# halajun/diasss

Hardware: AMD Instinct MI355X
Metric: sonar frames/sec end-to-end (extract+match+LM solve) (higher is better)
Workload: dtype u8/int32 (extract, match) + f64 (geo gate, LM); 1 GPU; 200 synthetic 2000x1024 frames, dense all-pairs; frames=200, pings=2000, bins=1024, pairs=19900

## Files before the change

diasss_amd/csrc/dsss_ctx.hip:

```cpp
#include "dsss_internal.h"
#include "dsss_pg_sym.h"
#include <algorithm>
#include <chrono>
#include <thread>
#include <atomic>
#include <cstdlib>

void dsss_prof_flush(dsss_ctx* c)
{
    if (!c || c->prof.pending.empty()) return;
    hipStreamSynchronize(c->stream);
    for (const dsss_prof::rec& r : c->prof.pending) {
        float ms = 0;
        if (hipEventElapsedTime(&ms, r.e0, r.e1) == hipSuccess) { c->prof.ms[r.k] += ms; c->prof.launches[r.k] += r.nl; }
        c->prof.pool.push_back(r.e0); c->prof.pool.push_back(r.e1);
    }
    c->prof.pending.clear();
}

dsss_switches dsss_switches_read()
{
    dsss_switches sw;
    if (const char* v = getenv("DSSS_EX_SCRATCH_MB")) sw.ex_scratch_mb = (size_t)std::max(1, atoi(v));
    if (const char* v = getenv("DSSS_EX_UPLOAD_BATCH")) sw.ex_upload_batch = std::max(1, atoi(v));
    sw.ex_verbose = getenv("DSSS_EX_VERBOSE") != nullptr;
    if (const char* v = getenv("DSSS_FS_THREADS")) sw.fs_threads = atoi(v);
    if (const char* v = getenv("DSSS_MT_GRID")) sw.mt_grid = atoi(v) != 0;
    sw.sift_hist_dump = getenv("DSSS_SIFT_HIST_DUMP");
    if (const char* v = getenv("DSSS_REG_PEAKS")) sw.reg_peaks_host = strcmp(v, "host") == 0;
    return sw;
}

extern "C" {

void dsss_mask_params_default(dsss_mask_params* p) { p->factor = 2.5; p->width = 10; p->r = 6; p->side = 150; }
void dsss_orb_params_default(dsss_orb_params* p) { p->nfeatures = 2000; p->scale = 1.2f; p->nlevels = 6; p->ini_th = 12; p->min_th = 7; p->descriptor = DSSS_DESC_ORB; }
void dsss_match_params_default(dsss_match_params* p)
{
    p->use_l2 = 0; p->radius = 8; p->bound_same = 88; p->bound_diff = 80; p->l2_bound = 350; p->ratio = 0.35;
    p->scc_iters = 1000; p->pix_err = 2.5; p->merge_thr = 2.5;
}
void dsss_pg_params_default(dsss_pg_params* p)
{
    p->max_iters = 100; p->rel_tol = 1e-5; p->abs_tol = 1e-5; p->lambda0 = 1e-5; p->lambda_factor = 10;
    p->lambda_max = 1e5; p->min_fidelity = 1e-3; p->add_noise = 1;
}

const char* dsss_strerror(int code)
{
    switch (code) {
    case DSSS_OK: return "ok";
    case DSSS_E_NODEVICE: return "no HIP device (libdsss has no CPU fallback)";
    case DSSS_E_ARG: return "bad argument";
    case DSSS_E_HIP: return "HIP runtime error";
    case DSSS_E_STATE: return "call order violated";
    case DSSS_E_CAPACITY: return "buffer too small";
    case DSSS_E_NUMERIC: return "numerical failure";
    case DSSS_E_COMM: return "communicator / RCCL failure";
    default: return "unknown error";
    }
}
const char* dsss_last_error(const dsss_ctx* c) { return c ? c->err.c_str() : "null context"; }

static int kcap_for(const dsss_orb_params& op) { return ((op.nfeatures + 3 * op.nlevels + 63) / 64 + 1) * 64; }

int dsss_create(int device, int max_frames, dsss_ctx** out)
{
    if (!out || max_frames <= 0) return DSSS_E_ARG;
    int ndev = 0;
    if (hipGetDeviceCount(&ndev) != hipSuccess || ndev <= 0 || device < 0 || device >= ndev) return DSSS_E_NODEVICE;
    if (hipSetDevice(device) != hipSuccess) return DSSS_E_NODEVICE;
    dsss_ctx* c = new dsss_ctx();
    c->device = device;
    dsss_mask_params_default(&c->mp); dsss_orb_params_default(&c->op);
    dsss_match_params_default(&c->mt); dsss_pg_params_default(&c->pg);
    c->max_frames = max_frames;
    c->frames.resize(max_frames);
    c->kcap = kcap_for(c->op);
    if (hipStreamCreateWithFlags(&c->stream, hipStreamNonBlocking) != hipSuccess) { delete c; return DSSS_E_HIP; }
    hipEventCreate(&c->prof.e0); hipEventCreate(&c->prof.e1);
    int prio_lo = 0, prio_hi = 0;
    (void)hipDeviceGetStreamPriorityRange(&prio_lo, &prio_hi);
    for (int i = 0; i < 4; ++i) {
        if (i == 1 && prio_hi != prio_lo) { if (hipStreamCreateWithPriority(&c->xs[i], hipStreamNonBlocking, prio_hi) != hipSuccess) { (void)hipGetLastError(); c->xs[i] = nullptr; } }
        if (!c->xs[i]) hipStreamCreateWithFlags(&c->xs[i], hipStreamNonBlocking);
        hipEventCreateWithFlags(&c->xev[i], hipEventDisableTiming);
    }
    for (int i = 0; i < DSSS_MAX_LEVELS; ++i) { hipEventCreateWithFlags(&c->ex_lev_ev[i], hipEventDisableTiming); hipEventCreateWithFlags(&c->ex_cmp_ev[i], hipEventDisableTiming); }
    for (int i = 0; i < 3; ++i) hipEventCreateWithFlags(&c->ex_side_ev[i], hipEventDisableTiming);
    hipEventCreateWithFlags(&c->xev_main, hipEventDisableTiming);
    *out = c;
    return DSSS_OK;
}

static std::array<dsss_fam_slot, 2> pack_family(dsss_frame& f, size_t pack = 0) { return {{ dsss_slot(f.d_pack, pack * sizeof(double)), dsss_slot(f.h_pack, pack * sizeof(double), DSSS_PINNED) }}; }
static std::array<dsss_fam_slot, 2> gbatch_family(dsss_geo_batch& G, size_t total = 0) { return {{ dsss_slot(G.d, total * sizeof(double)), dsss_slot(G.h, total * sizeof(double), DSSS_PINNED) }}; }
static std::array<dsss_fam_slot, 7> store_family(dsss_ctx* c)
{
    const size_t F = (size_t)c->max_frames, K = (size_t)c->kcap;
    return {{ dsss_slot(c->kps, F * K * sizeof(dsss_kp)), dsss_slot(c->desc, F * K * 32), dsss_slot(c->geo, F * K * 2 * sizeof(double)), dsss_slot(c->nkp_dev, F * sizeof(int)),
              dsss_slot(c->rows_dev, F * sizeof(int)), dsss_slot(c->cols_dev, F * sizeof(int)), dsss_slot(c->bbox_dev, F * 4 * sizeof(double)) }};
}

static void free_frame(dsss_frame& f)
{
    dsss_family_release(f.pack_cap, pack_family(f));
    hipFree(f.mask);
    if (f.pack_ev) hipEventDestroy(f.pack_ev);
    for (int l = 0; l < DSSS_MAX_LEVELS; ++l) hipFree(f.lvl[l]);
    const unsigned long long epoch = f.epoch;
    f = dsss_frame();
    f.epoch = epoch;
// ... 720 lines not shown
```

diasss_amd/csrc/dsss_internal.h:

```cpp
#pragma once
#include <hip/hip_runtime.h>
#include <cstdint>
#include <cstdio>
#include <cstring>
#include <cmath>
#include <cassert>
#include <array>
#include <string>
#include <utility>
#include <vector>
#include "../../include/dsss.h"

#define DSSS_MAX_LEVELS 8
#define DSSS_PI_REF 3.14159265359

struct dsss_ctx;
int dsss_hip_fail(dsss_ctx* c, hipError_t e, const char* file, int line, const char* call);
int dsss_alloc_fail(dsss_ctx* c, hipError_t e, const char* name, const char* step, size_t bytes);

inline hipError_t dsss_mem_alloc(void** p, size_t bytes, bool pinned) { return pinned ? hipHostMalloc(p, bytes, hipHostMallocDefault) : hipMalloc(p, bytes); }
inline void dsss_mem_free(void* p, bool pinned) { if (p) { if (pinned) (void)hipHostFree(p); else (void)hipFree(p); } }

struct dsss_buf {
    void* p = nullptr; size_t cap = 0; const char* const name; const bool pinned;
// ... 140 lines not shown
    dsss_prof prof;
};

#define DSSS_FAIL(ctx, code, ...) do { char _b[512]; snprintf(_b, sizeof _b, __VA_ARGS__); (ctx)->err = _b; return (code); } while (0)
#define HIPCHK(ctx, call) do { hipError_t _e = (call); if (_e != hipSuccess) return dsss_hip_fail((ctx), _e, __FILE__, __LINE__, #call); } while (0)
inline int dsss_hip_fail(dsss_ctx* c, hipError_t e, const char* file, int line, const char* call)
{
    char b[512]; snprintf(b, sizeof b, "%s:%d %s -> %s", file, line, call, hipGetErrorString(e));
    c->err = b; return DSSS_E_HIP;
}

inline int dsss_alloc_fail(dsss_ctx* c, hipError_t e, const char* name, const char* step, size_t bytes)
{
    char b[512]; snprintf(b, sizeof b, "%s: %s (%zu bytes) -> %s", name, step, bytes, hipGetErrorString(e));
    c->err = b; return DSSS_E_HIP;
}

inline int dsss_buf::reserve(dsss_ctx* c, size_t need_bytes, size_t alloc_bytes)
{
    if (cap >= need_bytes) return DSSS_OK;
    hipError_t e = p ? hipStreamSynchronize(c->stream) : hipSuccess;
    if (e != hipSuccess) { release(); return dsss_alloc_fail(c, e, name, "hipStreamSynchronize before the old block goes", alloc_bytes); }
    release();
    void* q = nullptr;
    if ((e = dsss_mem_alloc(&q, alloc_bytes, pinned)) != hipSuccess) return dsss_alloc_fail(c, e, name, pinned ? "hipHostMalloc" : "hipMalloc", alloc_bytes);
    p = q; cap = alloc_bytes;
    return DSSS_OK;
}
inline int dsss_buf::reserve_keep(dsss_ctx* c, size_t need_bytes, size_t alloc_bytes, size_t keep_bytes)
{
    if (cap >= need_bytes) return DSSS_OK;
    hipError_t e = p ? hipStreamSynchronize(c->stream) : hipSuccess;
    if (e != hipSuccess) return dsss_alloc_fail(c, e, name, "hipStreamSynchronize before the old block goes", alloc_bytes);
    dsss_buf nw(name, pinned);
    if ((e = dsss_mem_alloc(&nw.p, alloc_bytes, pinned)) != hipSuccess) { nw.p = nullptr; return dsss_alloc_fail(c, e, name, pinned ? "hipHostMalloc" : "hipMalloc", alloc_bytes); }
    nw.cap = alloc_bytes;
    if (keep_bytes > 0 && p && (e = hipMemcpy(nw.p, p, keep_bytes, hipMemcpyDeviceToDevice)) != hipSuccess) return dsss_alloc_fail(c, e, name, "copy of the kept prefix", keep_bytes);
    *this = std::move(nw);
    return DSSS_OK;
}
template <class Fam> int dsss_family_alloc(dsss_ctx* c, const char* name, size_t& cap, size_t new_cap, const Fam& fam)
{
    bool any = false;
    for (const dsss_fam_slot& s : fam) any = any || *s.pp != nullptr;
    hipError_t e = any ? hipStreamSynchronize(c->stream) : hipSuccess;
    dsss_family_release(cap, fam);
    if (e != hipSuccess) return dsss_alloc_fail(c, e, name, "hipStreamSynchronize before the old blocks go", 0);
    for (const dsss_fam_slot& s : fam) {
        void* q = nullptr;
        if ((e = dsss_mem_alloc(&q, s.bytes, s.pinned)) != hipSuccess) { dsss_family_release(cap, fam); return dsss_alloc_fail(c, e, name, s.pinned ? "hipHostMalloc" : "hipMalloc", s.bytes); }
        *s.pp = q;
    }
    cap = new_cap;
    return DSSS_OK;
}

struct dsss_scope {
    dsss_ctx* c; int k; int nl; hipEvent_t e0 = nullptr, e1 = nullptr;
    static hipEvent_t take(dsss_ctx* c) {
        hipEvent_t e = nullptr;
        if (!c->prof.pool.empty()) { e = c->prof.pool.back(); c->prof.pool.pop_back(); } else hipEventCreate(&e);
        return e;
    }
    dsss_scope(dsss_ctx* c_, int k_, double work = 0, int launches = 1) : c(c_), k(k_), nl(launches) {
        if (c->prof.on) { c->prof.work[k] += work; e0 = take(c); e1 = take(c); hipEventRecord(e0, c->stream); }
    }
    ~dsss_scope() {
        if (e0) {
            hipEventRecord(e1, c->stream);
            c->prof.pending.push_back({ k, nl, e0, e1 });
            if (c->prof.pending.size() >= 16384) dsss_prof_flush(c);
        }
    }
};

struct dsss_switches {
    size_t ex_scratch_mb = 24576;
    int ex_upload_batch = 8;
    bool ex_verbose = false;
    int fs_threads = 0;
    bool mt_grid = true;
    const char* sift_hist_dump = nullptr;
    bool reg_peaks_host = false;
};
dsss_switches dsss_switches_read();

void dsss_extract_eager(dsss_ctx* c, const int* ids, int n, const dsss_switches& sw);
int dsss_ensure_store(dsss_ctx* c);
int dsss_ensure_sift_store(dsss_ctx* c);
struct ex_frame;
void dsss_launch_sift_desc(dsss_ctx* c, hipStream_t st, const ex_frame* d_exf, int kcap, int nb, const char* hist_dump);
int dsss_frame_geo_bbox(dsss_ctx* c, int id);
int dsss_bboxes_enqueue(dsss_ctx* c);
int dsss_sync_bboxes(dsss_ctx* c);
int dsss_frame_kp_geo(dsss_ctx* c, int id, int n);
int dsss_mt_reserve_pair_index(dsss_ctx* c, size_t npairs);
int dsss_mt_reserve_pair_match(dsss_ctx* c, size_t npairs);
int dsss_mt_reserve_rows(dsss_ctx* c, size_t n);
int dsss_mt_upload_ptr_tables(dsss_ctx* c);
void dsss_mt_clear_results(dsss_ctx* c);
void dsss_mt_free(dsss_ctx* c);
void dsss_pg_free(dsss_ctx* c);
void dsss_comm_free(dsss_ctx* c);
void dsss_canvas_free_all(dsss_ctx* c);
int dsss_comm_rank(const dsss_ctx* c);
int dsss_comm_world(const dsss_ctx* c);
int dsss_comm_allreduce(dsss_ctx* c, double* dev, size_t n, hipStream_t st);
int dsss_comm_allgather(dsss_ctx* c, void* recv_dev, size_t bytes_per_rank, hipStream_t st);

__host__ __device__ inline void dsss_sincos(double x, double* s, double* c)
{
    const double invpio2 = 6.36619772367581382433e-01;
    const double pio2_1 = 1.57079632673412561417e+00;
    const double pio2_1t = 6.07710050650619224932e-11;
    double k = rint(x * invpio2);
    double r = (x - k * pio2_1) - k * pio2_1t;
    double z = r * r;
    double ps = 1.58969099521155010221e-10;
    ps = ps * z + -2.50507602534068634195e-08;
    ps = ps * z + 2.75573137070700676789e-06;
    ps = ps * z + -1.98412698298579493134e-04;
    ps = ps * z + 8.33333333332248946124e-03;
    ps = ps * z + -1.66666666666666324348e-01;
    double sr = r + (r * z) * ps;
    double pc = -1.13596475577881948265e-11;
    pc = pc * z + 2.08757232129817482790e-09;
    pc = pc * z + -2.75573143513906633035e-07;
    pc = pc * z + 2.48015872894767294178e-05;
    pc = pc * z + -1.38888888888741095749e-03;
    pc = pc * z + 4.16666666666666019037e-02;
    double cr = (1.0 - 0.5 * z) + (z * z) * pc;
    long long q = ((long long)k) & 3;
    if (q == 0) { *s = sr; *c = cr; }
    else if (q == 1) { *s = cr; *c = -sr; }
    else if (q == 2) { *s = -sr; *c = -cr; }
    else { *s = -cr; *c = sr; }
}

__host__ __device__ inline void dsss_geo_side(const double* P, bool starboard, double* s, double* c)
{
    dsss_sincos(starboard ? P[2] + DSSS_PI_REF / 2 : P[2] - DSSS_PI_REF / 2, s, c);
}
__host__ __device__ inline int dsss_geo_index(int M, int col)
{
    int half = M / 2, idx;
    if (col >= half) idx = col - half;
    else { idx = half - col; if (idx > half - 1) idx = half - 1; }
    return idx;
}
__host__ __device__ inline void dsss_geo_bin(const double* P, const double* gr, int M, int col, double s, double c, double* x, double* y)
{
    const int idx = dsss_geo_index(M, col);
    *x = (P[3] - 0.0) + gr[idx] * c;
    *y = (P[4] - 0.0) + gr[idx] * s;
}
__host__ __device__ inline void dsss_geo_at(const double* pose6, const double* gr, int M, int row, int col,
                                            double* x, double* y)
{
    const double* P = pose6 + (size_t)row * 6;
    double s, c;
    dsss_geo_side(P, col >= M / 2, &s, &c);
    dsss_geo_bin(P, gr, M, col, s, c, x, y);
}
__host__ __device__ inline void dsss_rotate_row(const double* row, double cx, double cy, double theta, double s, double c, double* out)
{
    out[0] = row[0]; out[1] = row[1]; out[5] = row[5];
// ... 8 lines not shown
```

diasss_amd/csrc/dsss_lc.hip:

```cpp
#include "dsss_internal.h"
#include "dsss_pose.h"
#include "dsss_lm.h"
#include <algorithm>

#define MR 16
#define MD 15

struct mini_prob {
    pose_t prior, odo;
    double sig_prior[6], sig_odo[6], sig_s[2], sig_t[2];
    double slant_s, slant_t;
};
struct mini_val { double L[3]; pose_t X1, X2; };

#define LG 16
#define LS 16
#define LIDX(i, k) ((k) * LS + (i) + 1)
struct lc_lds { double J[MR * LS]; double H[MD * LS]; double r[MR]; mini_prob m; mini_val v, nv; };

__device__ inline void lc_bcast_pose(const pose_t& mine, int src, pose_t* out)
{
#pragma unroll
    for (int k = 0; k < 9; ++k) out->R[k] = __shfl(mine.R[k], src, LG);
#pragma unroll
    for (int k = 0; k < 3; ++k) out->t[k] = __shfl(mine.t[k], src, LG);
}
__device__ inline void lc_select_pose(bool second, const pose_t& a, const pose_t& b, pose_t* out)
{
#pragma unroll
    for (int k = 0; k < 9; ++k) out->R[k] = second ? b.R[k] : a.R[k];
#pragma unroll
    for (int k = 0; k < 3; ++k) out->t[k] = second ? b.t[k] : a.t[k];
}
__device__ static void mini_lin(const mini_prob& m, const mini_val& v, double* r, double* J, int lane)
{
    const bool hb = (lane & 8) != 0;
    const bool wr = J && (lane & 7) == 0;
    if (J) {
#pragma unroll
        for (int c2 = 0; c2 < LS; ++c2) J[lane * LS + c2] = 0.0;
        __builtin_amdgcn_wave_barrier();
    }
    pose_t t1, t2, E; double xi[6], rr[6];
    const pose_t* P = hb ? &v.X1 : &m.prior;
    const pose_t* Q = hb ? &v.X2 : &v.X1;
    pose_between(P, Q, &t1);
    pose_between(&m.odo, &t1, &t2);
    lc_select_pose(hb, t1, t2, &E);
    pose_log(&E, xi);
#pragma unroll
    for (int i = 0; i < 6; ++i) { const double sg = hb ? m.sig_odo[i] : m.sig_prior[i]; rr[i] = xi[i] / sg; }
    if (!J) {
#pragma unroll
        for (int i = 0; i < 6; ++i) { r[i] = __shfl(rr[i], 0, LG); r[6 + i] = __shfl(rr[i], 8, LG); }
    } else if (wr) {
#pragma unroll
        for (int i = 0; i < 6; ++i) r[(hb ? 6 : 0) + i] = rr[i];
    }
    if (J) {
        pose_t hi; double Ad[36];
        pose_inverse(&t1, &hi);
        pose_adjoint(&hi, Ad);
        if (wr && !hb) {
#pragma unroll
            for (int i = 0; i < 6; ++i) J[i * LS + 3 + i] = 1.0 / m.sig_prior[i];
        }
        if (wr && hb) {
#pragma unroll
            for (int i = 0; i < 6; ++i) {
#pragma unroll
                for (int j = 0; j < 6; ++j) J[(6 + i) * LS + 3 + j] = -Ad[6 * i + j] / m.sig_odo[i];
                J[(6 + i) * LS + 9 + i] = 1.0 / m.sig_odo[i];
            }
        }
    }
    double ee[2], H1[6], H2[12], r2[2];
    const pose_t* X = hb ? &v.X2 : &v.X1;
    const double slant = hb ? m.slant_t : m.slant_s;
    const double sg0 = hb ? m.sig_t[0] : m.sig_s[0], sg1 = hb ? m.sig_t[1] : m.sig_s[1];
    sss_factor(v.L, X, slant, 0.0, ee, J ? H1 : nullptr, H2);
    r2[0] = ee[0] / sg0; r2[1] = ee[1] / sg1;
    if (!J) {
#pragma unroll
        for (int i = 0; i < 2; ++i) { r[12 + i] = __shfl(r2[i], 0, LG); r[14 + i] = __shfl(r2[i], 8, LG); }
    }
    if (wr) {
        const int row0 = hb ? 14 : 12, col0 = hb ? 9 : 3;
        r[row0] = r2[0]; r[row0 + 1] = r2[1];
#pragma unroll
        for (int i = 0; i < 2; ++i) {
            const double sg = i ? sg1 : sg0;
#pragma unroll
            for (int j = 0; j < 3; ++j) J[(row0 + i) * LS + j] = H1[3 * i + j] / sg;
#pragma unroll
            for (int j = 0; j < 6; ++j) J[(row0 + i) * LS + col0 + j] = H2[6 * i + j] / sg;
        }
    }
    if (J) __builtin_amdgcn_wave_barrier();
}
__device__ static __noinline__ double mini_err(const mini_prob& m, const mini_val& v, int lane)
{
    double r[MR];
    mini_lin(m, v, r, nullptr, lane);
    double s = 0;
#pragma unroll
    for (int i = 0; i < MR; ++i) s += r[i] * r[i];
    return 0.5 * s;
}
__device__ static double normal_eq(const double* J, const double* r, double* H, int lane)
{
    double g = 0;
    if (lane < MD) {
        double ca[MR];
#pragma unroll
        for (int k = 0; k < MR; ++k) ca[k] = J[k * LS + lane];
#pragma unroll
        for (int k = 0; k < MR; ++k) g += ca[k] * r[k];
        for (int b2 = 0; b2 < MD; ++b2) {
            double t = 0;
#pragma unroll
            for (int k = 0; k < MR; ++k) t += ca[k] * J[k * LS + b2];
            if (b2 <= lane) H[lane * LS + b2] = t;
            __builtin_amdgcn_sched_barrier(0);
        }
    }
    __builtin_amdgcn_wave_barrier();
    return g;
}
__device__ static int chol15(const double* H, double lambda, double* L, int lane)
{
    double row[MD];
    const int li = lane < MD ? lane : MD - 1;
#pragma unroll
    for (int j = 0; j < MD; ++j) row[j] = j <= li ? H[li * LS + j] + (j == li ? lambda : 0.0) : 0.0;
    int bad = 0;
#pragma unroll
    for (int j = 0; j < MD; ++j) {
        double sacc = row[j];
#pragma unroll
        for (int k = 0; k < MD; ++k) if (k < j) sacc -= row[k] * L[LIDX(j, k)];
        const double dj = __shfl(sacc, j, LG);
        if (!(dj > 0) || !isfinite(dj)) { bad = 1; break; }
        const double dq = sqrt(dj);
        row[j] = li == j ? dq : sacc / dq;
        if (lane < MD && li >= j) L[LIDX(li, j)] = row[j];
        __builtin_amdgcn_wave_barrier();
        __builtin_amdgcn_sched_barrier(0);
    }
    return bad;
}
__device__ static void chol15_solve(const double* L, double* b)
{
#pragma unroll
    for (int i = 0; i < MD; ++i) {
        double sacc = b[i];
#pragma unroll
        for (int k = 0; k < MD; ++k) if (k < i) sacc -= L[LIDX(i, k)] * b[k];
        b[i] = sacc / L[LIDX(i, i)];
        __builtin_amdgcn_sched_barrier(0);
    }
#pragma unroll
    for (int i = MD - 1; i >= 0; --i) {
        double sacc = b[i];
#pragma unroll
        for (int k = 0; k < MD; ++k) if (k > i) sacc -= L[LIDX(k, i)] * b[k];
        b[i] = sacc / L[LIDX(i, i)];
        __builtin_amdgcn_sched_barrier(0);
    }
}

__device__ inline void lc_comp_pose(bool on, pose_t* C)
{
    const double flipv[3] = { 0, 0, DSSS_PI_REF };
    pose_identity(C); if (on) so3_exp(flipv, C->R);
}
__device__ inline void lc_sss_sigmas(double slant, double* sig) { sig[0] = 0.1; sig[1] = slant * (0.1 * DSSS_PI_REF / 180); }
__device__ inline void lc_landmark_start(const double* geo_s, const double* geo_t, double z_s, double alt_s, double z_t, double alt_t, double* L)
{
    L[0] = (geo_s[0] + geo_t[0]) / 2; L[1] = (geo_s[1] + geo_t[1]) / 2; L[2] = ((z_s - alt_s) + (z_t - alt_t)) / 2;
}

struct lc_tables { const double* const* __restrict__ alt; const double* const* __restrict__ gr; const double* const* __restrict__ pose; const int* __restrict__ cols; };
static lc_tables lc_tables_of(const dsss_ctx* c) { const int F = c->max_frames; return { c->d_ptrs, c->d_ptrs + F, c->d_ptrs + 2 * F, c->cols_dev }; }

__device__ inline void lc_setup(lc_lds& S, const lc_tables& T, const double* kp, int fs, int ft, int flip, int lane, double* geo)
{
    const double PI = DSSS_PI_REF;
    const double* pose_s = T.pose[fs]; const double* pose_t_ = T.pose[ft];
    const int id_s = (int)kp[0], id_t = (int)kp[3];
    const bool hb = (lane & 8) != 0;
    mini_prob m;
    m.slant_s = kp[2]; m.slant_t = kp[5]; lc_sss_sigmas(kp[2], m.sig_s); lc_sss_sigmas(kp[5], m.sig_t);
    pose_t Tp_s, Tp_t, Tp_st;
    {
        pose_t Pm, Cm, Tm;
        pose_from_rodrigues(hb ? pose_t_ + (size_t)id_t * 6 : pose_s + (size_t)id_s * 6, &Pm);
        lc_comp_pose(flip & (hb ? 2 : 1), &Cm);
        pose_compose(&Pm, &Cm, &Tm);
        lc_bcast_pose(Tm, 0, &Tp_s); lc_bcast_pose(Tm, 8, &Tp_t);
    }
    pose_between(&Tp_s, &Tp_t, &Tp_st);
    for (int k = 0; k < 6; ++k) m.sig_prior[k] = 0.000001;
    m.sig_odo[0] = 0.1 * PI / 180; m.sig_odo[1] = 0.1 * PI / 180; m.sig_odo[2] = 0.5 * PI / 180;
    m.sig_odo[3] = fabs(Tp_st.t[0] * 2); m.sig_odo[4] = fabs(Tp_st.t[1] / 10); m.sig_odo[5] = 0.1;
    for (int k = 3; k < 5; ++k) if (m.sig_odo[k] < 1e-9) m.sig_odo[k] = 1e-9;
    m.prior = Tp_s; m.odo = Tp_st;
    double gx, gy;
    dsss_geo_at(hb ? pose_t_ : pose_s, hb ? T.gr[ft] : T.gr[fs], hb ? T.cols[ft] : T.cols[fs], hb ? id_t : id_s, hb ? (int)kp[4] : (int)kp[1], &gx, &gy);
    geo[0] = __shfl(gx, 0, LG); geo[1] = __shfl(gy, 0, LG); geo[2] = __shfl(gx, 8, LG); geo[3] = __shfl(gy, 8, LG);
    mini_val v;
    lc_landmark_start(geo, geo + 2, pose_s[(size_t)id_s * 6 + 5], T.alt[fs][id_s], pose_t_[(size_t)id_t * 6 + 5], T.alt[ft][id_t], v.L);
    v.X1 = Tp_s; v.X2 = Tp_t;
    if (lane == 0) { S.m = m; S.v = v; }
    __builtin_amdgcn_wave_barrier();
}
__device__ inline lm_verdict lc_trial(lc_lds& S, const lm_rule& R, double g_mine, double lambda, double oldLin, double err, int lane, double* newErr)
{
    const lm_verdict refused = { false, false };
    if (chol15(S.H, lambda, S.H, lane) != 0) return refused;
    double d[MD];
#pragma unroll
    for (int a = 0; a < MD; ++a) d[a] = -__shfl(g_mine, a, LG);
    chol15_solve(S.H, d);
    double sk = S.r[lane];
#pragma unroll
    for (int a = 0; a < MD; ++a) sk += S.J[lane * LS + a] * d[a];
    double newLin = 0;
#pragma unroll
    for (int k = 0; k < MR; ++k) { const double t = __shfl(sk, k, LG); newLin += t * t; }
    newLin *= 0.5;
    if (!lm_descends(oldLin, newLin)) return refused;
    {
        const bool hb = (lane & 8) != 0;
        pose_t Xn; double dx[6];
        const pose_t* X = hb ? &S.v.X2 : &S.v.X1;
#pragma unroll
        for (int a = 0; a < 6; ++a) dx[a] = hb ? d[9 + a] : d[3 + a];
        pose_retract(X, dx, &Xn);
        if (lane == 0) { for (int a = 0; a < 3; ++a) S.nv.L[a] = S.v.L[a] + d[a]; S.nv.X1 = Xn; }
        if (lane == 8) S.nv.X2 = Xn;
        __builtin_amdgcn_wave_barrier();
    }
    *newErr = mini_err(S.m, S.nv, lane);
    return lm_judge(R, oldLin, newLin, err, *newErr);
}
__device__ inline void lc_take_trial(lc_lds& S, int lane)
{
    const double* src = reinterpret_cast<const double*>(&S.nv); double* dst = reinterpret_cast<double*>(&S.v);
    const double e0 = src[lane], e1 = lane + LG < (int)(sizeof(mini_val) / sizeof(double)) ? src[lane + LG] : 0.0;
    __builtin_amdgcn_wave_barrier();
    dst[lane] = e0; if (lane + LG < (int)(sizeof(mini_val) / sizeof(double))) dst[lane + LG] = e1;
    __builtin_amdgcn_wave_barrier();
}
__device__ inline int lc_lm(lc_lds& S, int lane, double* err_io)
{
    const lm_rule R = lm_gtsam_defaults();
    double lambda = 1e-5, err = *err_io, cur;
    int iters = 0;
    if (err > 0) do {
        cur = err;
        mini_lin(S.m, S.v, S.r, S.J, lane);
        const double g_mine = normal_eq(S.J, S.r, S.H, lane);
        double oldLin = 0;
#pragma unroll
        for (int k = 0; k < MR; ++k) oldLin += S.r[k] * S.r[k];
        oldLin *= 0.5;
        for (;;) {
            double newErr = 0;
            const lm_verdict v = lc_trial(S, R, g_mine, lambda, oldLin, err, lane, &newErr);
            if (v.success) { lc_take_trial(S, lane); err = newErr; lm_accepted(R, &lambda); ++iters; break; }
            if (v.stop || lm_refused(R, &lambda)) break;
        }
    } while (lm_continue(R, iters, cur, err));
    *err_io = err; return iters;
}
__device__ inline double lc_score(const lc_lds& S, const double* kp, const double* gr_t, int Mt, int flip, const double* geo, pose_t* new_pose)
{
    const double PI = DSSS_PI_REF;
    pose_t cq, cti;
    lc_comp_pose(flip & 2, &cq); pose_inverse(&cq, &cti);
    pose_compose(&S.v.X2, &cti, new_pose);
    const double x_o = geo[0] - geo[2], y_o = geo[1] - geo[3], ini = sqrt(x_o * x_o + y_o * y_o);
    double rpy[3]; pose_rpy(new_pose, rpy);
    const bool port = kp[4] < Mt / 2;
    const int gi = port ? Mt / 2 - (int)kp[4] : (int)kp[4] - Mt / 2;
    const double bearing = port ? rpy[2] + PI / 2 - PI : rpy[2] - PI / 2 - PI;
    const double lx = new_pose->t[0] + gr_t[gi] * cos(bearing), ly = new_pose->t[1] + gr_t[gi] * sin(bearing);
    const double x_n = geo[0] - lx, y_n = geo[1] - ly;
    return ini / sqrt(x_n * x_n + y_n * y_n) - 2;
}
__device__ inline void lc_marginal_var(lc_lds& S, int lane, double* var)
{
    mini_lin(S.m, S.v, S.r, S.J, lane);
    (void)normal_eq(S.J, S.r, S.H, lane);
    double var_mine = NAN;
    if (chol15(S.H, 0.0, S.H, lane) == 0) {
        double d[MD];
#pragma unroll
        for (int a = 0; a < MD; ++a) d[a] = (a == 9 + lane) ? 1.0 : 0.0;
        chol15_solve(S.H, d);
        var_mine = 0;
#pragma unroll
        for (int a = 9; a < MD; ++a) if (a == 9 + lane) var_mine = d[a];
    }
#pragma unroll
    for (int c2 = 0; c2 < 6; ++c2) var[c2] = __shfl(var_mine, c2, LG);
}
__device__ inline void lc_rel_pose(const lc_lds& S, int flip, const pose_t& new_pose, double* rel12)
{
    pose_t cq, csi, src, rel;
    lc_comp_pose(flip & 1, &cq); pose_inverse(&cq, &csi);
    pose_compose(&S.m.prior, &csi, &src); pose_between(&src, &new_pose, &rel);
    for (int a = 0; a < 9; ++a) rel12[a] = rel.R[a];
    for (int a = 0; a < 3; ++a) rel12[9 + a] = rel.t[a];
}

__global__ __launch_bounds__(64, 2) void lc_kernel(const double* __restrict__ kp7, int n, const int* __restrict__ kp7_pair, const uint8_t* __restrict__ kp7_flip,
                                                const int* __restrict__ act_s, const int* __restrict__ act_t, int single_s, int single_t, lc_tables T, dsss_lc* __restrict__ out)
{
    __shared__ lc_lds s_all[64 / LG];
    const int grp = threadIdx.x / LG, lane = threadIdx.x % LG;
    const int i = blockIdx.x * (64 / LG) + grp;
    if (i >= n) return;
    lc_lds& S = s_all[grp];
    const double* kp = kp7 + (size_t)i * 7;
    const int fs = kp7_pair ? act_s[kp7_pair[i]] : single_s, ft = kp7_pair ? act_t[kp7_pair[i]] : single_t;
    const int flip = kp7_flip[i];
    double geo[4]; dsss_lc o;
    lc_setup(S, T, kp, fs, ft, flip, lane, geo);
    o.pad_ = 0; o.err0 = o.err1 = mini_err(S.m, S.v, lane);
    o.iters = lc_lm(S, lane, &o.err1);
    pose_t new_pose;
    o.score = lc_score(S, kp, T.gr[ft], T.cols[ft], flip, geo, &new_pose);
    lc_marginal_var(S, lane, o.var);
    lc_rel_pose(S, flip, new_pose, o.rel);
    if (lane == 0) out[i] = o;
}

struct tri_frame { const double* pose; const double* alt; const double* gr; int M; };
struct tri_prob { pose_t Tp_s, Tp_t; double slant_s, slant_t, sig_s[2], sig_t[2], sig_p[3], ini[3]; };

__device__ inline void tri_setup(tri_prob& P, const double* kp, const tri_frame& s, const tri_frame& t, int flip, const double* q)
{
    if (q) {
        for (int k = 0; k < 9; ++k) { P.Tp_s.R[k] = q[k]; P.Tp_t.R[k] = q[12 + k]; }
        for (int k = 0; k < 3; ++k) { P.Tp_s.t[k] = q[9 + k]; P.Tp_t.t[k] = q[21 + k]; P.ini[k] = q[24 + k]; }
    } else {
        const int id_s = (int)kp[0], id_t = (int)kp[3];
        pose_t cps_s, cps_t, Ps, Pt;
        lc_comp_pose(flip & 1, &cps_s); lc_comp_pose(flip & 2, &cps_t);
        pose_from_rodrigues(s.pose + (size_t)id_s * 6, &Ps); pose_from_rodrigues(t.pose + (size_t)id_t * 6, &Pt);
        pose_compose(&Ps, &cps_s, &P.Tp_s); pose_compose(&Pt, &cps_t, &P.Tp_t);
        double geo_s[2], geo_t[2];
        dsss_geo_at(s.pose, s.gr, s.M, id_s, (int)kp[1], &geo_s[0], &geo_s[1]);
        dsss_geo_at(t.pose, t.gr, t.M, id_t, (int)kp[4], &geo_t[0], &geo_t[1]);
        lc_landmark_start(geo_s, geo_t, s.pose[(size_t)id_s * 6 + 5], s.alt[id_s], t.pose[(size_t)id_t * 6 + 5], t.alt[id_t], P.ini);
    }
    P.slant_s = kp[2]; P.slant_t = kp[5]; lc_sss_sigmas(kp[2], P.sig_s); lc_sss_sigmas(kp[5], P.sig_t);
    const double dx = P.Tp_s.t[0] - P.Tp_t.t[0], dy = P.Tp_s.t[1] - P.Tp_t.t[1];
    P.sig_p[0] = 10.0; P.sig_p[1] = 10.0; P.sig_p[2] = sqrt(dx * dx + dy * dy) / 100;
    if (P.sig_p[2] < 1e-9) P.sig_p[2] = 1e-9;
}
__device__ static void tri_lin(const tri_prob& P, const double* p, double* r, double* J)
{
    double ee[2], H1[6], H2[12];
    sss_factor(p, &P.Tp_s, P.slant_s, 0.0, ee, J ? H1 : nullptr, H2);
    for (int i = 0; i < 2; ++i) { r[i] = ee[i] / P.sig_s[i]; if (J) for (int j = 0; j < 3; ++j) J[i * 3 + j] = H1[3 * i + j] / P.sig_s[i]; }
    sss_factor(p, &P.Tp_t, P.slant_t, 0.0, ee, J ? H1 : nullptr, H2);
    for (int i = 0; i < 2; ++i) { r[2 + i] = ee[i] / P.sig_t[i]; if (J) for (int j = 0; j < 3; ++j) J[(2 + i) * 3 + j] = H1[3 * i + j] / P.sig_t[i]; }
    for (int i = 0; i < 3; ++i) { r[4 + i] = (p[i] - P.ini[i]) / P.sig_p[i]; if (J) for (int j = 0; j < 3; ++j) J[(4 + i) * 3 + j] = (i == j) ? 1.0 / P.sig_p[i] : 0.0; }
}
__device__ static double tri_err(const tri_prob& P, const double* p)
{
    double rr[7], t = 0;
    tri_lin(P, p, rr, nullptr); for (int k = 0; k < 7; ++k) t += rr[k] * rr[k];
    return 0.5 * t;
}
__device__ static int tri_chol3(double* A)
{
    for (int j = 0; j < 3; ++j) {
        double d = A[j * 3 + j];
        for (int k = 0; k < j; ++k) d -= A[j * 3 + k] * A[j * 3 + k];
        if (!(d > 0) || !isfinite(d)) return -1;
        d = sqrt(d); A[j * 3 + j] = d;
        for (int i = j + 1; i < 3; ++i) { double t = A[i * 3 + j]; for (int k = 0; k < j; ++k) t -= A[i * 3 + k] * A[j * 3 + k]; A[i * 3 + j] = t / d; }
    }
    return 0;
}
__device__ inline void tri_lm(const tri_prob& P, double* p)
{
    const lm_rule R = lm_gtsam_defaults();
    double lambda = 1e-5, err = tri_err(P, p), cur;
    int iters = 0;
    if (err > 0) do {
        cur = err;
        double r[7], J[21], H[9], g[3];
        tri_lin(P, p, r, J);
        for (int a = 0; a < 3; ++a) {
            double t = 0; for (int k = 0; k < 7; ++k) t += J[k * 3 + a] * r[k];
            g[a] = t;
            for (int b = 0; b < 3; ++b) { double u = 0; for (int k = 0; k < 7; ++k) u += J[k * 3 + a] * J[k * 3 + b]; H[a * 3 + b] = u; }
        }
        double oldLin = 0; for (int k = 0; k < 7; ++k) oldLin += r[k] * r[k];
        oldLin *= 0.5;
        for (;;) {
            double A[9], d[3], np_[3] = { 0, 0, 0 }, newErr = 0, newLin = 0;
            lm_verdict v = { false, false };
            for (int a = 0; a < 9; ++a) A[a] = H[a];
            for (int a = 0; a < 3; ++a) { A[a * 3 + a] += lambda; d[a] = -g[a]; }
            if (tri_chol3(A) == 0) {
                for (int a = 0; a < 3; ++a) { double t = d[a]; for (int k = 0; k < a; ++k) t -= A[a * 3 + k] * d[k]; d[a] = t / A[a * 3 + a]; }
                for (int a = 2; a >= 0; --a) { double t = d[a]; for (int k = a + 1; k < 3; ++k) t -= A[k * 3 + a] * d[k]; d[a] = t / A[a * 3 + a]; }
                for (int k = 0; k < 7; ++k) { double t = r[k]; for (int a = 0; a < 3; ++a) t += J[k * 3 + a] * d[a]; newLin += t * t; }
                newLin *= 0.5;
                if (lm_descends(oldLin, newLin)) {
                    for (int a = 0; a < 3; ++a) np_[a] = p[a] + d[a];
                    newErr = tri_err(P, np_);
                    v = lm_judge(R, oldLin, newLin, err, newErr);
                }
            }
            if (v.success) { for (int a = 0; a < 3; ++a) p[a] = np_[a]; err = newErr; lm_accepted(R, &lambda); ++iters; break; }
            if (v.stop || lm_refused(R, &lambda)) break;
        }
    } while (lm_continue(R, iters, cur, err));
}
__global__ __launch_bounds__(64) void tri_kernel(const double* __restrict__ kp7, int n, const uint8_t* __restrict__ flips, tri_frame fs, tri_frame ft,
                                                 const double* __restrict__ explicit27, double* __restrict__ out7)
{
    const int i = blockIdx.x * 64 + threadIdx.x;
    if (i >= n) return;
    const double* kp = kp7 + (size_t)i * 7;
    tri_prob P;
    tri_setup(P, kp, fs, ft, flips ? flips[i] : 0, explicit27 ? explicit27 + (size_t)i * 27 : nullptr);
    double p[3] = { P.ini[0], P.ini[1], P.ini[2] };
    tri_lm(P, p);
    double* o = out7 + (size_t)i * 7;
    o[0] = p[0]; o[1] = p[1]; o[2] = p[2];
    double e[2];
    sss_factor(p, &P.Tp_s, P.slant_s, 0.0, e, nullptr, nullptr); o[3] = fabs(e[0]); o[4] = fabs(e[1]);
    sss_factor(p, &P.Tp_t, P.slant_t, 0.0, e, nullptr, nullptr); o[5] = fabs(e[0]); o[6] = fabs(e[1]);
}

static int check_kp7_rows(dsss_ctx* c, const dsss_frame& fs, const dsss_frame& ft, const double* rows, int n, int pair)
{
    for (int i = 0; i < n; ++i) {
        const double* k = rows + (size_t)i * 7;
        if (k[0] >= 0 && k[0] < fs.N && k[3] >= 0 && k[3] < ft.N && k[1] >= 1 && k[1] < fs.M && k[4] >= 1 && k[4] < ft.M) continue;
        char who[32] = ""; if (pair >= 0) snprintf(who, sizeof who, "pair %d ", pair);
        DSSS_FAIL(c, DSSS_E_ARG, "%skp7 row %d: ping/bin outside the frames (%g,%g | %g,%g)", who, i, k[0], k[1], k[3], k[4]);
    }
    return DSSS_OK;
}
static void lc_sticky_flags(const dsss_frame& fs, const dsss_frame& ft, const double* rows, int n, uint8_t* flip)
{
    uint8_t f = 0;
    for (int i = 0; i < n; ++i) {
        const double* k = rows + (size_t)i * 7;
        if (dsss_yaw_flips(fs.h_geo[(size_t)(int)k[0] * 6 + 2])) f |= 1;
        if (dsss_yaw_flips(ft.h_geo[(size_t)(int)k[3] * 6 + 2])) f |= 2;
        flip[i] = f;
    }
}
static int lc_one_list(dsss_ctx* c, int id_s, int id_t, const double* kp7, int n, std::vector<double>* h, std::vector<uint8_t>* flip)
{
    if (id_s < 0 || id_s >= c->max_frames || id_t < 0 || id_t >= c->max_frames) DSSS_FAIL(c, DSSS_E_ARG, "frame id out of range");
    const dsss_frame &fs = c->frames[id_s], &ft = c->frames[id_t];
    if (!fs.has_geom || !ft.has_geom) DSSS_FAIL(c, DSSS_E_STATE, "frames need dsss_frame_set first");
    if (!fs.h_geo || !ft.h_geo) DSSS_FAIL(c, DSSS_E_STATE, "host copy of the DR poses missing");
    if (n == 0) return DSSS_OK;
    HIPCHK(c, hipSetDevice(c->device));
    h->resize((size_t)n * 7); flip->resize(n);
    HIPCHK(c, hipMemcpy(h->data(), kp7, h->size() * sizeof(double), hipMemcpyDefault));
    if (const int rc = check_kp7_rows(c, fs, ft, h->data(), n, -1)) return rc;
    lc_sticky_flags(fs, ft, h->data(), n, flip->data());
    return DSSS_OK;
}
static int lc_launch(dsss_ctx* c, const double* kp7, int n, const int* kp7_pair, const uint8_t* kp7_flip, const int* act_s, const int* act_t, int single_s, int single_t,
                     dsss_lc* out)
{
    dsss_scope sc(c, DSSS_K_LC);
    hipLaunchKernelGGL(lc_kernel, dim3((n + 3) / 4), dim3(64), 0, c->stream, kp7, n, kp7_pair, kp7_flip, act_s, act_t, single_s, single_t, lc_tables_of(c), out);
    HIPCHK(c, hipGetLastError());
    return DSSS_OK;
}
static int tri_run(dsss_ctx* c, const double* kp7, int n, const uint8_t* h_flip, const tri_frame& fs, const tri_frame& ft, const double* in27, double* out7)
{
    const size_t nd = (size_t)n * (7 + 7 + (in27 ? 27 : 0));
    dsss_buf d("triangulation rows, inputs and results");
    if (const int rc = d.reserve(c, nd * sizeof(double) + (h_flip ? (size_t)n : 0))) return rc;
    double* d_kp7 = d.as<double>(); double* d_out = d_kp7 + (size_t)n * 7; double* d_in = in27 ? d_out + (size_t)n * 7 : nullptr;
    uint8_t* d_flip = h_flip ? reinterpret_cast<uint8_t*>(d_kp7 + nd) : nullptr;
    HIPCHK(c, hipMemcpyAsync(d_kp7, kp7, (size_t)n * 7 * sizeof(double), hipMemcpyDefault, c->stream));
    if (d_in) HIPCHK(c, hipMemcpyAsync(d_in, in27, (size_t)n * 27 * sizeof(double), hipMemcpyDefault, c->stream));
    if (d_flip) HIPCHK(c, hipMemcpyAsync(d_flip, h_flip, (size_t)n, hipMemcpyHostToDevice, c->stream));
    hipLaunchKernelGGL(tri_kernel, dim3((n + 63) / 64), dim3(64), 0, c->stream, (const double*)d_kp7, n, (const uint8_t*)d_flip, fs, ft, (const double*)d_in, d_out);
    HIPCHK(c, hipGetLastError());
    HIPCHK(c, hipMemcpyAsync(out7, d_out, (size_t)n * 7 * sizeof(double), hipMemcpyDeviceToHost, c->stream));
    HIPCHK(c, hipStreamSynchronize(c->stream));
    return DSSS_OK;
}
static tri_frame tri_frame_of(const dsss_frame& f) { return { f.pose6, f.alt, f.gr, f.M }; }

extern "C" {

int dsss_lc_solve_all(dsss_ctx* c)
{
    if (!c) return DSSS_E_ARG;
    HIPCHK(c, hipSetDevice(c->device));
    const int n = c->total_kp7;
    c->has_lc = false;
    if (const int rc = c->lcs.reserve(c, (size_t)n * sizeof(dsss_lc), ((size_t)n + 1024) * sizeof(dsss_lc))) return rc;
    if (n > 0)
        if (const int rc = lc_launch(c, c->kp7, n, c->kp7_pair, c->kp7_flip, c->act_s, c->act_t, 0, 0, c->lcs.as<dsss_lc>())) return rc;
    c->has_lc = true; ++c->lc_gen;
    return DSSS_OK;
}

int dsss_lc_get(dsss_ctx* c, int pair, dsss_lc* out, int cap, int* nout)
{
    if (!c) return DSSS_E_ARG;
    if (pair < 0 || pair >= c->npairs) DSSS_FAIL(c, DSSS_E_ARG, "pair %d out of range", pair);
    if (!c->has_lc) DSSS_FAIL(c, DSSS_E_STATE, "dsss_lc_solve_all has not run");
    const int a = c->pair_active[pair];
    const int n = a < 0 ? 0 : c->h_kp7_off[a + 1] - c->h_kp7_off[a];
    if (nout) *nout = n;
    if (n == 0 || !out) return DSSS_OK;
    if (cap < n) DSSS_FAIL(c, DSSS_E_CAPACITY, "caller capacity %d < %d", cap, n);
    HIPCHK(c, hipStreamSynchronize(c->stream));
    HIPCHK(c, hipMemcpy(out, c->lcs.as<dsss_lc>() + c->h_kp7_off[a], (size_t)n * sizeof(dsss_lc), hipMemcpyDeviceToHost));
    return DSSS_OK;
}

int dsss_lc_solve_pairs(dsss_ctx* c, const int* src_ids, const int* tgt_ids, int npairs, const double* kp7, const int* pair_off)
{
    if (!c || npairs < 0 || (npairs > 0 && (!src_ids || !tgt_ids || !pair_off))) return DSSS_E_ARG;
    dsss_mt_clear_results(c);
    HIPCHK(c, hipSetDevice(c->device));
    const int n = npairs > 0 ? pair_off[npairs] : 0;
    if (n < 0 || (n > 0 && !kp7)) return DSSS_E_ARG;
    for (int p = 0; p < npairs; ++p) {
        const int s = src_ids[p], t = tgt_ids[p];
        if (s < 0 || s >= c->max_frames || t < 0 || t >= c->max_frames || s == t) DSSS_FAIL(c, DSSS_E_ARG, "pair %d: bad frame ids (%d,%d)", p, s, t);
        if (!c->frames[s].has_geom || !c->frames[t].has_geom) DSSS_FAIL(c, DSSS_E_STATE, "pair %d: frames need dsss_frame_set first", p);
        if (pair_off[p + 1] < pair_off[p] || pair_off[0] != 0) DSSS_FAIL(c, DSSS_E_ARG, "pair_off does not start at 0 or is not ascending at pair %d", p);
    }
    int rc = dsss_sync_bboxes(c); if (rc) return rc;
    if ((rc = dsss_mt_upload_ptr_tables(c))) return rc;
    std::vector<double> h((size_t)n * 7);
    if (n > 0) HIPCHK(c, hipMemcpy(h.data(), kp7, h.size() * sizeof(double), hipMemcpyDefault));
    std::vector<int> h_pair(n); std::vector<uint8_t> h_flip(n);
    for (int p = 0; p < npairs && n > 0; ++p) {
        const dsss_frame &fs = c->frames[src_ids[p]], &ft = c->frames[tgt_ids[p]];
        const int o = pair_off[p], np = pair_off[p + 1] - o;
        if (!fs.h_geo || !ft.h_geo) DSSS_FAIL(c, DSSS_E_STATE, "pair %d: host copy of the DR poses missing", p);
        if ((rc = check_kp7_rows(c, fs, ft, h.data() + (size_t)o * 7, np, p))) return rc;
        lc_sticky_flags(fs, ft, h.data() + (size_t)o * 7, np, h_flip.data() + o);
        std::fill(h_pair.begin() + o, h_pair.begin() + o + np, p);
    }
    if (n > 0) {
        HIPCHK(c, hipStreamSynchronize(c->stream));
        if ((rc = dsss_mt_reserve_pair_index(c, npairs)) || (rc = dsss_mt_reserve_rows(c, n))) return rc;
        HIPCHK(c, hipMemcpy(c->act_s, src_ids, npairs * sizeof(int), hipMemcpyHostToDevice)); HIPCHK(c, hipMemcpy(c->act_t, tgt_ids, npairs * sizeof(int), hipMemcpyHostToDevice));
        HIPCHK(c, hipMemcpy(c->kp7_off, pair_off, (npairs + 1) * sizeof(int), hipMemcpyHostToDevice));
        HIPCHK(c, hipMemcpy(c->kp7, h.data(), h.size() * sizeof(double), hipMemcpyHostToDevice));
        HIPCHK(c, hipMemcpy(c->kp7_pair, h_pair.data(), (size_t)n * sizeof(int), hipMemcpyHostToDevice)); HIPCHK(c, hipMemcpy(c->kp7_flip, h_flip.data(), (size_t)n, hipMemcpyHostToDevice));
    }
    c->npairs = c->nactive = npairs; c->total_kp7 = n;
    c->pair_s.assign(src_ids, src_ids + npairs); c->pair_t.assign(tgt_ids, tgt_ids + npairs);
    c->pair_active.resize(npairs); for (int p = 0; p < npairs; ++p) c->pair_active[p] = p;
    c->h_row_off.assign(npairs + 1, 0); if (npairs > 0) c->h_kp7_off.assign(pair_off, pair_off + npairs + 1);
    return dsss_lc_solve_all(c);
}

int dsss_lc_solve(dsss_ctx* c, int id_s, int id_t, const double* kp7, int n, dsss_lc* out)
{
    if (!c || n < 0 || (n > 0 && (!kp7 || !out))) return DSSS_E_ARG;
    std::vector<double> h; std::vector<uint8_t> flip;
    int rc = lc_one_list(c, id_s, id_t, kp7, n, &h, &flip); if (rc || n == 0) return rc;
    if ((rc = dsss_sync_bboxes(c))) return rc;
    if ((rc = dsss_mt_upload_ptr_tables(c))) return rc;
    dsss_buf d_kp7("dsss_lc_solve kp7"), d_flip("dsss_lc_solve flags"), d_out("dsss_lc_solve results");
    if ((rc = d_kp7.reserve(c, h.size() * sizeof(double))) || (rc = d_flip.reserve(c, flip.size())) || (rc = d_out.reserve(c, (size_t)n * sizeof(dsss_lc)))) return rc;
    HIPCHK(c, hipMemcpyAsync(d_kp7.p, h.data(), h.size() * sizeof(double), hipMemcpyHostToDevice, c->stream));
    HIPCHK(c, hipMemcpyAsync(d_flip.p, flip.data(), flip.size(), hipMemcpyHostToDevice, c->stream));
    if ((rc = lc_launch(c, d_kp7.as<double>(), n, nullptr, d_flip.as<uint8_t>(), nullptr, nullptr, id_s, id_t, d_out.as<dsss_lc>()))) return rc;
    HIPCHK(c, hipMemcpyAsync(out, d_out.p, (size_t)n * sizeof(dsss_lc), hipMemcpyDeviceToHost, c->stream));
    HIPCHK(c, hipStreamSynchronize(c->stream));
    return DSSS_OK;
}

int dsss_triangulate(dsss_ctx* c, int id_s, int id_t, const double* kp7, int n, double* out7)
{
    if (!c || n < 0 || (n > 0 && (!kp7 || !out7))) return DSSS_E_ARG;
    std::vector<double> h; std::vector<uint8_t> flip;
    const int rc = lc_one_list(c, id_s, id_t, kp7, n, &h, &flip); if (rc || n == 0) return rc;
    return tri_run(c, h.data(), n, flip.data(), tri_frame_of(c->frames[id_s]), tri_frame_of(c->frames[id_t]), nullptr, out7);
}

int dsss_triangulate_poses(dsss_ctx* c, const double* kp7, const double* in27, int n, double* out7)
{
    if (!c || n < 0 || (n > 0 && (!kp7 || !in27 || !out7))) return DSSS_E_ARG;
    if (n == 0) return DSSS_OK;
    HIPCHK(c, hipSetDevice(c->device));
    return tri_run(c, kp7, n, nullptr, tri_frame{}, tri_frame{}, in27, out7);
}

}
```

Measured before the change: 9841 frames/s.

## Fuse LM error evaluation with relinearization and spread Jacobian writes across lanes

Adds a per-pair LM loop in which each trial point is linearized once and the same residuals serve as both the new error and the next linearization. On rejection it restores the saved Jacobian blocks from spare H storage instead of recomputing them, and the final marginal-variance step reuses the last linearization. Jacobian row writes are distributed across lanes with select chains rather than done serially by the writer lanes. This cuts the separate mini_err and relinearization passes per iteration, at the cost of extra LDS save/restore traffic and more complex control flow. The old path stays available behind an environment switch.

```diff
diff --git a/diasss_amd/csrc/dsss_ctx.hip b/diasss_amd/csrc/dsss_ctx.hip
--- a/diasss_amd/csrc/dsss_ctx.hip
+++ b/diasss_amd/csrc/dsss_ctx.hip
@@ -28,6 +28,7 @@
     if (const char* v = getenv("DSSS_MT_GRID")) sw.mt_grid = atoi(v) != 0;
     sw.sift_hist_dump = getenv("DSSS_SIFT_HIST_DUMP");
     if (const char* v = getenv("DSSS_REG_PEAKS")) sw.reg_peaks_host = strcmp(v, "host") == 0;
+    if (const char* v = getenv("DSSS_LC_EVAL")) sw.lc_eval_twice = strcmp(v, "twice") == 0;
     return sw;
 }
 
diff --git a/diasss_amd/csrc/dsss_internal.h b/diasss_amd/csrc/dsss_internal.h
--- a/diasss_amd/csrc/dsss_internal.h
+++ b/diasss_amd/csrc/dsss_internal.h
@@ -246,6 +246,7 @@
     bool mt_grid = true;
     const char* sift_hist_dump = nullptr;
     bool reg_peaks_host = false;
+    bool lc_eval_twice = false;
 };
 dsss_switches dsss_switches_read();
 
diff --git a/diasss_amd/csrc/dsss_lc.hip b/diasss_amd/csrc/dsss_lc.hip
--- a/diasss_amd/csrc/dsss_lc.hip
+++ b/diasss_amd/csrc/dsss_lc.hip
@@ -61,16 +61,18 @@
         pose_t hi; double Ad[36];
         pose_inverse(&t1, &hi);
         pose_adjoint(&hi, Ad);
-        if (wr && !hb) {
-#pragma unroll
-            for (int i = 0; i < 6; ++i) J[i * LS + 3 + i] = 1.0 / m.sig_prior[i];
-        }
-        if (wr && hb) {
-#pragma unroll
-            for (int i = 0; i < 6; ++i) {
-#pragma unroll
-                for (int j = 0; j < 6; ++j) J[(6 + i) * LS + 3 + j] = -Ad[6 * i + j] / m.sig_odo[i];
-                J[(6 + i) * LS + 9 + i] = 1.0 / m.sig_odo[i];
+        const int q = lane & 7;
+        if (q < 6) {
+            const double sg = hb ? m.sig_odo[q] : m.sig_prior[q];
+            J[((hb ? 6 : 0) + q) * LS + (hb ? 9 : 3) + q] = 1.0 / sg;
+            if (hb) {
+#pragma unroll
+                for (int j = 0; j < 6; ++j) {
+                    double a = Ad[j];
+#pragma unroll
+                    for (int i = 1; i < 6; ++i) a = q == i ? Ad[6 * i + j] : a;
+                    J[(6 + q) * LS + 3 + j] = -a / sg;
+                }
             }
         }
     }
@@ -84,17 +86,18 @@
 #pragma unroll
         for (int i = 0; i < 2; ++i) { r[12 + i] = __shfl(r2[i], 0, LG); r[14 + i] = __shfl(r2[i], 8, LG); }
     }
-    if (wr) {
-        const int row0 = hb ? 14 : 12, col0 = hb ? 9 : 3;
-        r[row0] = r2[0]; r[row0 + 1] = r2[1];
-#pragma unroll
-        for (int i = 0; i < 2; ++i) {
-            const double sg = i ? sg1 : sg0;
-#pragma unroll
-            for (int j = 0; j < 3; ++j) J[(row0 + i) * LS + j] = H1[3 * i + j] / sg;
-#pragma unroll
-            for (int j = 0; j < 6; ++j) J[(row0 + i) * LS + col0 + j] = H2[6 * i + j] / sg;
-        }
+    if (J) {
+        const int row0 = hb ? 14 : 12, col0 = hb ? 9 : 3, q = lane & 7;
+        if (wr) { r[row0] = r2[0]; r[row0 + 1] = r2[1]; }
+        double a0 = H1[0], a1 = H1[3];
+#pragma unroll
+        for (int k = 1; k < 8; ++k) {
+            a0 = q == k ? (k < 3 ? H1[k] : H2[k - 3]) : a0;
+            a1 = q == k ? (k < 3 ? H1[3 + k] : H2[6 + k - 3]) : a1;
+        }
+        const int col = q < 3 ? q : col0 + q - 3;
+        J[row0 * LS + col] = a0 / sg0; J[(row0 + 1) * LS + col] = a1 / sg1;
+        if (q == 0) { J[row0 * LS + col0 + 5] = H2[5] / sg0; J[(row0 + 1) * LS + col0 + 5] = H2[11] / sg1; }
     }
     if (J) __builtin_amdgcn_wave_barrier();
 }
@@ -214,10 +217,9 @@
     if (lane == 0) { S.m = m; S.v = v; }
     __builtin_amdgcn_wave_barrier();
 }
-__device__ inline lm_verdict lc_trial(lc_lds& S, const lm_rule& R, double g_mine, double lambda, double oldLin, double err, int lane, double* newErr)
-{
-    const lm_verdict refused = { false, false };
-    if (chol15(S.H, lambda, S.H, lane) != 0) return refused;
+__device__ inline bool lc_step(lc_lds& S, double g_mine, double lambda, double oldLin, int lane, double* newLin_out)
+{
+    if (chol15(S.H, lambda, S.H, lane) != 0) return false;
     double d[MD];
 #pragma unroll
     for (int a = 0; a < MD; ++a) d[a] = -__shfl(g_mine, a, LG);
@@ -229,7 +231,8 @@
 #pragma unroll
     for (int k = 0; k < MR; ++k) { const double t = __shfl(sk, k, LG); newLin += t * t; }
     newLin *= 0.5;
-    if (!lm_descends(oldLin, newLin)) return refused;
+    *newLin_out = newLin;
+    if (!lm_descends(oldLin, newLin)) return false;
     {
         const bool hb = (lane & 8) != 0;
         pose_t Xn; double dx[6];
@@ -241,6 +244,13 @@
         if (lane == 8) S.nv.X2 = Xn;
         __builtin_amdgcn_wave_barrier();
     }
+    return true;
+}
+__device__ inline lm_verdict lc_trial(lc_lds& S, const lm_rule& R, double g_mine, double lambda, double oldLin, double err, int lane, double* newErr)
+{
+    const lm_verdict refused = { false, false };
+    double newLin = 0;
+    if (!lc_step(S, g_mine, lambda, oldLin, lane, &newLin)) return refused;
     *newErr = mini_err(S.m, S.nv, lane);
     return lm_judge(R, oldLin, newLin, err, *newErr);
 }
@@ -273,6 +283,63 @@
         }
     } while (lm_continue(R, iters, cur, err));
     *err_io = err; return iters;
+}
+__device__ inline void lc_lin_keep(lc_lds& S, int lane, bool keep)
+{
+    const bool sss = lane >= 12;
+    const int n = lane < 6 ? 0 : sss ? 9 : 6;
+    const int q = lane < 6 ? 0 : sss ? lane - 12 : lane - 2;
+    const int c0 = lane >= 14 ? 9 : 3;
+    __builtin_amdgcn_wave_barrier();
+#pragma unroll
+    for (int j = 0; j < 9; ++j)
+        if (j < n) {
+            double& a = S.J[lane * LS + (sss ? (j < 3 ? j : c0 + j - 3) : 3 + j)];
+            double& b = S.H[q * LS + q + 1 + j];
+            if (keep) b = a; else a = b;
+        }
+    __builtin_amdgcn_wave_barrier();
+}
+__device__ inline int lc_lm_once(lc_lds& S, int lane, double* err0, double* err1)
+{
+    const lm_rule R = lm_gtsam_defaults();
+    double lambda = 1e-5, err = 0, cur = 0, oldLin = 0, newLin = 0, g_mine = 0, r_mine = 0;
+    int iters = 0;
+    bool trial = false;
+    for (;;) {
+        mini_lin(S.m, trial ? S.nv : S.v, S.r, S.J, lane);
+        double e = 0;
+#pragma unroll
+        for (int k = 0; k < MR; ++k) e += S.r[k] * S.r[k];
+        e *= 0.5;
+        bool relin = true;
+        if (!trial) {
+            *err0 = err = e;
+            if (!(err > 0)) break;
+        } else {
+            const lm_verdict v = lm_judge(R, oldLin, newLin, err, e);
+            if (v.success) {
+                lc_take_trial(S, lane); err = e; lm_accepted(R, &lambda); ++iters;
+                if (!lm_continue(R, iters, cur, err)) break;
+            } else {
+                lc_lin_keep(S, lane, false); S.r[lane] = r_mine;
+                __builtin_amdgcn_wave_barrier();
+                if (v.stop || lm_refused(R, &lambda)) break;
+                relin = false;
+            }
+        }
+        if (relin) {
+            cur = err;
+            g_mine = normal_eq(S.J, S.r, S.H, lane);
+            oldLin = e;
+        }
+        bool step;
+        while (!(step = lc_step(S, g_mine, lambda, oldLin, lane, &newLin)) && !lm_refused(R, &lambda)) {}
+        if (!step) break;
+        r_mine = S.r[lane]; lc_lin_keep(S, lane, true);
+        trial = true;
+    }
+    *err1 = err; return iters;
 }
 __device__ inline double lc_score(const lc_lds& S, const double* kp, const double* gr_t, int Mt, int flip, const double* geo, pose_t* new_pose)
 {
@@ -289,9 +356,9 @@
     const double x_n = geo[0] - lx, y_n = geo[1] - ly;
     return ini / sqrt(x_n * x_n + y_n * y_n) - 2;
 }
-__device__ inline void lc_marginal_var(lc_lds& S, int lane, double* var)
-{
-    mini_lin(S.m, S.v, S.r, S.J, lane);
+__device__ inline void lc_marginal_var(lc_lds& S, int lane, bool relin, double* var)
+{
+    if (relin) mini_lin(S.m, S.v, S.r, S.J, lane);
     (void)normal_eq(S.J, S.r, S.H, lane);
     double var_mine = NAN;
     if (chol15(S.H, 0.0, S.H, lane) == 0) {
@@ -315,6 +382,7 @@
     for (int a = 0; a < 3; ++a) rel12[9 + a] = rel.t[a];
 }
 
+template <bool ONCE>
 __global__ __launch_bounds__(64, 2) void lc_kernel(const double* __restrict__ kp7, int n, const int* __restrict__ kp7_pair, const uint8_t* __restrict__ kp7_flip,
                                                 const int* __restrict__ act_s, const int* __restrict__ act_t, int single_s, int single_t, lc_tables T, dsss_lc* __restrict__ out)
 {
@@ -328,11 +396,12 @@
     const int flip = kp7_flip[i];
     double geo[4]; dsss_lc o;
     lc_setup(S, T, kp, fs, ft, flip, lane, geo);
-    o.pad_ = 0; o.err0 = o.err1 = mini_err(S.m, S.v, lane);
-    o.iters = lc_lm(S, lane, &o.err1);
+    o.pad_ = 0;
+    if constexpr (ONCE) o.iters = lc_lm_once(S, lane, &o.err0, &o.err1);
+    else { o.err0 = o.err1 = mini_err(S.m, S.v, lane); o.iters = lc_lm(S, lane, &o.err1); }
     pose_t new_pose;
     o.score = lc_score(S, kp, T.gr[ft], T.cols[ft], flip, geo, &new_pose);
-    lc_marginal_var(S, lane, o.var);
+    lc_marginal_var(S, lane, !ONCE, o.var);
     lc_rel_pose(S, flip, new_pose, o.rel);
     if (lane == 0) out[i] = o;
 }
@@ -475,11 +544,12 @@
     lc_sticky_flags(fs, ft, h->data(), n, flip->data());
     return DSSS_OK;
 }
-static int lc_launch(dsss_ctx* c, const double* kp7, int n, const int* kp7_pair, const uint8_t* kp7_flip, const int* act_s, const int* act_t, int single_s, int single_t,
+static int lc_launch(dsss_ctx* c, bool twice, const double* kp7, int n, const int* kp7_pair, const uint8_t* kp7_flip, const int* act_s, const int* act_t, int single_s, int single_t,
                      dsss_lc* out)
 {
     dsss_scope sc(c, DSSS_K_LC);
-    hipLaunchKernelGGL(lc_kernel, dim3((n + 3) / 4), dim3(64), 0, c->stream, kp7, n, kp7_pair, kp7_flip, act_s, act_t, single_s, single_t, lc_tables_of(c), out);
+    hipLaunchKernelGGL(twice ? lc_kernel<false> : lc_kernel<true>, dim3((n + 3) / 4), dim3(64), 0, c->stream, kp7, n, kp7_pair, kp7_flip, act_s, act_t, single_s, single_t,
+                       lc_tables_of(c), out);
     HIPCHK(c, hipGetLastError());
     return DSSS_OK;
 }
@@ -501,19 +571,24 @@
 }
 static tri_frame tri_frame_of(const dsss_frame& f) { return { f.pose6, f.alt, f.gr, f.M }; }
 
-extern "C" {
-
-int dsss_lc_solve_all(dsss_ctx* c)
-{
-    if (!c) return DSSS_E_ARG;
+static int lc_solve_all(dsss_ctx* c, const dsss_switches& sw)
+{
     HIPCHK(c, hipSetDevice(c->device));
     const int n = c->total_kp7;
     c->has_lc = false;
     if (const int rc = c->lcs.reserve(c, (size_t)n * sizeof(dsss_lc), ((size_t)n + 1024) * sizeof(dsss_lc))) return rc;
     if (n > 0)
-        if (const int rc = lc_launch(c, c->kp7, n, c->kp7_pair, c->kp7_flip, c->act_s, c->act_t, 0, 0, c->lcs.as<dsss_lc>())) return rc;
+        if (const int rc = lc_launch(c, sw.lc_eval_twice, c->kp7, n, c->kp7_pair, c->kp7_flip, c->act_s, c->act_t, 0, 0, c->lcs.as<dsss_lc>())) return rc;
     c->has_lc = true; ++c->lc_gen;
     return DSSS_OK;
+}
+
+extern "C" {
+
+int dsss_lc_solve_all(dsss_ctx* c)
+{
+    if (!c) return DSSS_E_ARG;
+    return lc_solve_all(c, dsss_switches_read());
 }
 
 int dsss_lc_get(dsss_ctx* c, int pair, dsss_lc* out, int cap, int* nout)
@@ -534,6 +609,7 @@
 int dsss_lc_solve_pairs(dsss_ctx* c, const int* src_ids, const int* tgt_ids, int npairs, const double* kp7, const int* pair_off)
 {
     if (!c || npairs < 0 || (npairs > 0 && (!src_ids || !tgt_ids || !pair_off))) return DSSS_E_ARG;
+    const dsss_switches sw = dsss_switches_read();
     dsss_mt_clear_results(c);
     HIPCHK(c, hipSetDevice(c->device));
     const int n = npairs > 0 ? pair_off[npairs] : 0;
@@ -569,12 +645,13 @@
     c->pair_s.assign(src_ids, src_ids + npairs); c->pair_t.assign(tgt_ids, tgt_ids + npairs);
     c->pair_active.resize(npairs); for (int p = 0; p < npairs; ++p) c->pair_active[p] = p;
     c->h_row_off.assign(npairs + 1, 0); if (npairs > 0) c->h_kp7_off.assign(pair_off, pair_off + npairs + 1);
-    return dsss_lc_solve_all(c);
+    return lc_solve_all(c, sw);
 }
 
 int dsss_lc_solve(dsss_ctx* c, int id_s, int id_t, const double* kp7, int n, dsss_lc* out)
 {
     if (!c || n < 0 || (n > 0 && (!kp7 || !out))) return DSSS_E_ARG;
+    const dsss_switches sw = dsss_switches_read();
     std::vector<double> h; std::vector<uint8_t> flip;
     int rc = lc_one_list(c, id_s, id_t, kp7, n, &h, &flip); if (rc || n == 0) return rc;
     if ((rc = dsss_sync_bboxes(c))) return rc;
@@ -583,7 +660,7 @@
     if ((rc = d_kp7.reserve(c, h.size() * sizeof(double))) || (rc = d_flip.reserve(c, flip.size())) || (rc = d_out.reserve(c, (size_t)n * sizeof(dsss_lc)))) return rc;
     HIPCHK(c, hipMemcpyAsync(d_kp7.p, h.data(), h.size() * sizeof(double), hipMemcpyHostToDevice, c->stream));
     HIPCHK(c, hipMemcpyAsync(d_flip.p, flip.data(), flip.size(), hipMemcpyHostToDevice, c->stream));
-    if ((rc = lc_launch(c, d_kp7.as<double>(), n, nullptr, d_flip.as<uint8_t>(), nullptr, nullptr, id_s, id_t, d_out.as<dsss_lc>()))) return rc;
+    if ((rc = lc_launch(c, sw.lc_eval_twice, d_kp7.as<double>(), n, nullptr, d_flip.as<uint8_t>(), nullptr, nullptr, id_s, id_t, d_out.as<dsss_lc>()))) return rc;
     HIPCHK(c, hipMemcpyAsync(out, d_out.p, (size_t)n * sizeof(dsss_lc), hipMemcpyDeviceToHost, c->stream));
     HIPCHK(c, hipStreamSynchronize(c->stream));
     return DSSS_OK;
```

After: 9840 frames/s. About the same (-0.0%).
